# mulns/AccFlow

Measured on AMD Instinct MI355X. Metric: frame-pairs/s (estimator pair-evals/s), AccFlow(RAFT) 7-frame 480x1024 backward accumulation, higher is better.
Workload: dtype f32 (direct-kernel operands split into 2 fp16 terms - activations kept pre-split in HBM as fp16 hi+lo, 4 B per element; other kernels 3 bf16 terms; f32 accumulate); 1 GPU; AccFlow(RAFT) 7-frame 480x1024, 12 GRU iters, 1 sequence(s)/GPU/step (BASELINE.json configs[2]; configs[3] when n_gpus=8); parallelism=1 rank, no process group: no collective runs, weights=deterministic random init (no checkpoints offline)

## Files before the change

### accflow_amd/backward.py

```python
import torch

from . import _lib, ops, profiler
from .ops import _check, _p, _plane4, _stream


def _chw(t):
    return t.shape[1] * t.shape[2] * t.shape[3]


def act_backward(dy, y, act, out=None):
    lib = _lib.load()
    if out is None:
        out = torch.empty(tuple(dy.shape), dtype=torch.float32, device=dy.device)
    if tuple(dy.shape) != tuple(y.shape) or tuple(out.shape) != tuple(y.shape):
        raise RuntimeError("act_backward: shapes differ")
    _check(lib.accflow_act_backward_f32(_p(dy), _plane4(dy, "dy"), _p(y), _plane4(y, "y"), _p(out), _plane4(out, "dx"),
                                        dy.shape[0], _chw(dy), int(act), _stream()), "accflow_act_backward_f32")
    return out


def add_(dst, src):
    lib = _lib.load()
    if tuple(dst.shape) != tuple(src.shape):
        raise RuntimeError("add_: shapes differ")
    _check(lib.accflow_add_f32(_p(dst), _plane4(dst, "dst"), _p(src), _plane4(src, "src"), dst.shape[0], _chw(dst), _stream()),
           "accflow_add_f32")
    return dst


def l1_grad(pred, gt, scale):
    lib = _lib.load()
    pred, gt = ops._dense(pred, "pred"), ops._dense(gt, "gt")
    out = torch.empty_like(pred)
    _check(lib.accflow_l1_grad_f32(_p(pred), _p(gt), _p(out), pred.numel(), float(scale), _stream()), "accflow_l1_grad_f32")
    return out


def blend_backward(dy, f1, f2, m):
    lib = _lib.load()
    dy, f1, f2, m = (ops._dense(t, n) for t, n in ((dy, "dy"), (f1, "f1"), (f2, "f2"), (m, "m")))
    B, C, H, W = f1.shape
    df1, df2 = torch.empty_like(f1), torch.empty_like(f1)
    dm = torch.empty((B, 1, H, W), dtype=torch.float32, device=f1.device)
    _check(lib.accflow_blend_backward_f32(_p(dy), _p(f1), _p(f2), _p(m), _p(df1), _p(df2), _p(dm), B, C, H * W, _stream()),
           "accflow_blend_backward_f32")
    return df1, df2, dm


def convex_upsample_backward(dup, flow, mask):
    lib = _lib.load()
    dup, flow, mask = ops._dense(dup, "dup"), ops._dense(flow, "flow"), ops._dense(mask, "mask")
    B, _, H8, W8 = flow.shape
    if tuple(dup.shape) != (B, 2, 8 * H8, 8 * W8) or tuple(mask.shape) != (B, 576, H8, W8):
        raise RuntimeError("convex_upsample_backward: dup (B,2,8H8,8W8), mask (B,576,H8,W8)")
    dflow, dmask = torch.empty_like(flow), torch.empty_like(mask)
    _check(lib.accflow_convex_upsample_backward_f32(_p(dup), _p(flow), _p(mask), _p(dflow), _p(dmask), B, H8, W8, _stream()),
           "accflow_convex_upsample_backward_f32")
    return dflow, dmask


def conv_wgrad(x, dy, KH, KW, stride=1, padding=(0, 0), bias=True):
    lib = _lib.load()
    xbs, dbs = _plane4(x, "x"), _plane4(dy, "dy")
    B, Cin, H, W = x.shape
    Cout = dy.shape[1]
    pH, pW = (padding, padding) if isinstance(padding, int) else padding
    OH, OW = (H + 2 * pH - KH) // stride + 1, (W + 2 * pW - KW) // stride + 1
    if tuple(dy.shape) != (B, Cout, OH, OW):
        raise RuntimeError("conv_wgrad: dy is %s, expected %s" % (tuple(dy.shape), (B, Cout, OH, OW)))
    dw = torch.empty((Cout, Cin, KH, KW), dtype=torch.float32, device=x.device)
    db = torch.empty((Cout,), dtype=torch.float32, device=x.device) if bias else None
    tm = profiler.ACTIVE
    t0 = tm.begin() if tm is not None and tm.wants("conv_wgrad") else None
    _check(lib.accflow_conv_wgrad_f32(_p(x), xbs, _p(dy), dbs, _p(dw), _p(db), B, Cin, Cout, H, W, KH, KW, int(stride), int(pH),
                                      int(pW), _stream()), "accflow_conv_wgrad_f32")
    if t0 is not None:
        tm.end("conv_wgrad", t0, 2.0 * Cout * Cin * KH * KW * B * OH * OW, "wgrad Cin%d Cout%d k%dx%d s%d B%d %dx%d" % (
            Cin, Cout, KH, KW, stride, B, H, W))
    return dw, db


GRAD_CONV_MODE = "bf16x6"

_DGRAD_CACHE = {}


def _cached(deps, tag, build):
    if deps is None:
        return build()
    key = (tag, tuple(id(d) for d in deps))
    sig = tuple((d.data_ptr(), d._version, str(d.device)) for d in deps)
    hit = _DGRAD_CACHE.get(key)
    if hit is None or hit[0] != sig:
        hit = _DGRAD_CACHE[key] = [sig, build()]
    return hit[1]


def conv_dgrad(dy, weight, in_hw, stride=1, padding=(0, 0), out=None, deps=None):
    lib = _lib.load()
    pH, pW = (padding, padding) if isinstance(padding, int) else padding
    H, W = in_hw
    B = dy.shape[0]
    if callable(weight):
        weight = _cached(deps, "w", weight)
    Cout, Cin, KH, KW = weight.shape
    pad = (KH - 1 - pH, KW - 1 - pW)
    def make_pack():
        if ops.PACK_FUSED and Cin > 4:
            return ops.PackedConv(weight.detach().float(), None, stride=1, padding=pad, transpose_flip=True)
        return ops.PackedConv(weight.detach().float().transpose(0, 1).flip(2, 3).contiguous(), None, stride=1, padding=pad)
    pk = _cached(deps, ("pk", pad), make_pack)
    if stride != 1:
        Hd, Wd = H + 2 * pH - KH + 1, W + 2 * pW - KW + 1
        OH, OW = dy.shape[2:]
        g = torch.empty((B, Cout, Hd, Wd), dtype=torch.float32, device=dy.device)
        _check(lib.accflow_dilate_f32(_p(dy), _plane4(dy, "dy"), _p(g), B, Cout, OH, OW, Hd, Wd, int(stride), _stream()),
               "accflow_dilate_f32")
        dy = g
    with ops.conv_mode(GRAD_CONV_MODE):
        dx = ops.conv2d(pk, dy, out=out)
    if tuple(dx.shape[2:]) != (H, W):
        raise RuntimeError("conv_dgrad: got %s for an input of %s" % (tuple(dx.shape), (H, W)))
    return dx


def deform_conv_backward(x, offset, mask, weight, dy, need_dx=True, deps=None):
    lib = _lib.load()
    B, C, H, W = x.shape
    Cout, _, KH, KW = weight.shape
    T = KH * KW
    pH, pW = (KH - 1) // 2, (KW - 1) // 2
    cols = torch.empty((B, T * C, H, W), dtype=torch.float32, device=x.device)
    _check(lib.accflow_deform_columns_f32(_p(x), _plane4(x, "x"), _p(offset), _plane4(offset, "offset"), _p(mask),
                                          _plane4(mask, "dmask"), _p(cols), B, C, H, W, KH, KW, pH, pW, _stream()),
           "accflow_deform_columns_f32")
    dwz, db = conv_wgrad(cols, dy, 1, 1)
    dweight = dwz.reshape(Cout, KH, KW, C).permute(0, 3, 1, 2).contiguous()
    dcols = conv_dgrad(dy, lambda: weight.detach().float().permute(0, 2, 3, 1).reshape(Cout, T * C, 1, 1), (H, W),
                       deps=deps)
    dx = torch.empty((B, C, H, W), dtype=torch.float32, device=x.device)
    doff = torch.empty((B, 2 * T, H, W), dtype=torch.float32, device=x.device)
    dmsk = torch.empty((B, T, H, W), dtype=torch.float32, device=x.device)
    _check(lib.accflow_deform_conv_backward_f32(_p(x), _plane4(x, "x"), _p(offset), _plane4(offset, "offset"), _p(mask),
                                                _plane4(mask, "dmask"), _p(dcols), _p(dx), _plane4(dx, "dx"), _p(doff),
                                                _p(dmsk), B, C, H, W, KH, KW, pH, pW, _stream()),
           "accflow_deform_conv_backward_f32")
    return (dx if need_dx else None), doff, dmsk, dweight, db
```

### accflow_amd/csrc/conv2d_direct_kernel.h

```cpp
#pragma once
#include "conv_common.h"
#include <utility>

namespace {


#ifndef ACCFLOW_DIRECT_LEAN
#define ACCFLOW_DIRECT_LEAN 1
#endif
#ifndef ACCFLOW_DIRECT_LEAN_MAXSTEPS
#define ACCFLOW_DIRECT_LEAN_MAXSTEPS 0
#endif
#ifndef ACCFLOW_F16_PAIRMASK
#define ACCFLOW_F16_PAIRMASK 7
#endif
#ifndef ACCFLOW_DIRECT_KT_BUPFRONT
#define ACCFLOW_DIRECT_KT_BUPFRONT 0
#endif
#ifndef ACCFLOW_DIRECT_KT_WAVES
#define ACCFLOW_DIRECT_KT_WAVES 3
#endif
#ifndef ACCFLOW_DIRECT_SETPRIO
#define ACCFLOW_DIRECT_SETPRIO 0
#endif
template <class F, int... I>
__device__ __forceinline__ void dir_static_for_impl(std::integer_sequence<int, I...>, F&& f) {
  (f(std::integral_constant<int, I>{}), ...);
}
template <int N, class F>
__device__ __forceinline__ void dir_static_for(F&& f) { dir_static_for_impl(std::make_integer_sequence<int, N>{}, f); }

typedef int s16m_i32x4 __attribute__((ext_vector_type(4)));
__device__ __forceinline__ void s16m_load_a(u32x4& dst, unsigned voff, s16m_i32x4 desc, int soff) {
  asm volatile("buffer_load_dwordx4 %0, %1, %2, %3 offen" : "=v"(dst) : "v"(voff), "s"(desc), "s"(soff) : "memory");
}
template <int N>
__device__ __forceinline__ void s16m_wait_vm() {
  asm volatile("s_waitcnt vmcnt(%0)" : : "n"(N) : "memory");
  __builtin_amdgcn_sched_barrier(0);
}
__device__ __forceinline__ void s16m_wait_vm_but(int n) {
#define S16M_W(N) case N: s16m_wait_vm<N>(); break;
  switch (n) {
    S16M_W(1) S16M_W(2) S16M_W(3) S16M_W(4) S16M_W(5) S16M_W(6) S16M_W(7) S16M_W(8) S16M_W(9) S16M_W(10)
    S16M_W(11) S16M_W(12) S16M_W(13) S16M_W(14) S16M_W(15) S16M_W(16) S16M_W(17) S16M_W(18) S16M_W(19) S16M_W(20)
    S16M_W(21) S16M_W(22) S16M_W(23) S16M_W(24) S16M_W(25) S16M_W(26) S16M_W(27) S16M_W(28) S16M_W(29) S16M_W(30)
    default: s16m_wait_vm<0>();
  }
#undef S16M_W
}

template <bool F16>
__device__ __forceinline__ f32x16 dir_mfma(bf16x8 a, bf16x8 b, f32x16 c) {
  if constexpr (F16) return __builtin_amdgcn_mfma_f32_32x32x16_f16(__builtin_bit_cast(f16x8, a), __builtin_bit_cast(f16x8, b), c, 0, 0, 0);
  else return __builtin_amdgcn_mfma_f32_32x32x16_bf16(a, b, c, 0, 0, 0);
}

template <bool F16, class PixMap>
__device__ __forceinline__ void conv_epilogue_tapgemm(const accflow_conv_desc& d, f32x16 (&acc)[1][4], int cblk0, int wave,
                                                      int lane, int tid, int OHW, PixMap pixmap, float* red) {
  typedef float f32x4_ __attribute__((ext_vector_type(4)));
  typedef float f32x2_ __attribute__((ext_vector_type(2)));
  typedef _Float16 f16x2_ __attribute__((ext_vector_type(2)));
  const int l31 = lane & 31, kh = lane >> 5, lh4 = kh * 4;
  const int rowbase = cblk0 + wave * 32;
  const int R = d.tg_rows;
  const __amdgpu_buffer_rsrc_t r_b = __builtin_amdgcn_make_buffer_rsrc(const_cast<float*>(d.bias ? d.bias : d.wscale16), 0,
                                                                      d.bias ? d.Cout * 4 : 0, 0x00020000);
  const __amdgpu_buffer_rsrc_t r_s = __builtin_amdgcn_make_buffer_rsrc(const_cast<float*>(d.wscale16), 0, d.CoutPad * 4, 0x00020000);
  f32x4_ bv[4], sv[4];
#pragma unroll
  for (int m = 0; m < 4; ++m) {
    const int off = (rowbase + 8 * m + lh4) * 4;
    bv[m] = __builtin_bit_cast(f32x4_, __builtin_amdgcn_raw_buffer_load_b128(r_b, off, 0, 0));
    sv[m] = __builtin_bit_cast(f32x4_, __builtin_amdgcn_raw_buffer_load_b128(r_s, off, 0, 0));
  }
  const long long step_bytes2 = 2LL * d.tg_coutpad * 16, term_bytes2 = (long long)(d.Cout >> 4) * step_bytes2;
  const __amdgpu_buffer_rsrc_t r_w2 = __builtin_amdgcn_make_buffer_rsrc(const_cast<void*>(d.tg_w16), 0,
                                                                       (int)(unsigned)(2 * term_bytes2), 0x00020000);
  const unsigned av2 = (unsigned)((kh * d.tg_coutpad + l31) * 16);
  bf16x8 a2[2][2];
#pragma unroll
  for (int s = 0; s < 2; ++s)
#pragma unroll
    for (int t = 0; t < 2; ++t)
      a2[s][t] = __builtin_bit_cast(bf16x8, __builtin_amdgcn_raw_buffer_load_b128(
                                               r_w2, (int)av2, (int)(unsigned)(t * term_bytes2 + ((rowbase >> 4) + s) * step_bytes2), 0));
  constexpr float ASC16 = (float)(1 << ACCFLOW_F16_ASHIFT);
  bool bad16 = false;
#pragma unroll
  for (int tp = 0; tp < 4; ++tp) {
    f32x16 z2;
#pragma unroll
    for (int r = 0; r < 16; ++r) z2[r] = 0.0f;
#pragma unroll
    for (int s = 0; s < 2; ++s) {
      unsigned hi[4], lo[4];
#pragma unroll
      for (int e2 = 0; e2 < 4; ++e2) {
        const int m = 2 * s + (e2 >> 1), q = (2 * e2) & 3;
        float va = fmaf(acc[0][tp][4 * m + q], sv[m][q], bv[m][q]) + 0.0f;
        float vb = fmaf(acc[0][tp][4 * m + q + 1], sv[m][q + 1], bv[m][q + 1]) + 0.0f;
        va = fmaxf(va, 0.0f) * ASC16;
        vb = fmaxf(vb, 0.0f) * ASC16;
        bad16 |= !(va < 65520.0f) | !(vb < 65520.0f);
        const f32x2_ v2 = {va, vb};
        const f16x2_ hq = __builtin_convertvector(v2, f16x2_);
        const f32x2_ back = __builtin_convertvector(hq, f32x2_);
        const f32x2_ rest = {va - back[0], vb - back[1]};
        const f16x2_ lq = __builtin_convertvector(rest, f16x2_);
        hi[e2] = __builtin_bit_cast(unsigned, hq);
        lo[e2] = __builtin_bit_cast(unsigned, lq);
      }
      const u32x4 hv = {hi[0], hi[1], hi[2], hi[3]}, lv = {lo[0], lo[1], lo[2], lo[3]};
      const bf16x8 bh = __builtin_bit_cast(bf16x8, hv), bl = __builtin_bit_cast(bf16x8, lv);
      z2 = dir_mfma<F16>(a2[s][1], bh, z2);
      z2 = dir_mfma<F16>(a2[s][0], bl, z2);
      z2 = dir_mfma<F16>(a2[s][0], bh, z2);
    }
#pragma unroll
    for (int r = 0; r < 16; ++r) {
      const int row = 8 * (r >> 2) + lh4 + (r & 3);
      if (row < R) red[(wave * R + row) * (DIR_TH * DIR_TW) + tp * 32 + l31] = z2[r];
    }
  }
  if (bad16 && d.guard) atomicOr(d.guard, 1);
  __syncthreads();
  const long long obase = (long long)(cblk0 >> 7) * d.tg_out_ps;
  constexpr int NPX = DIR_TH * DIR_TW;
  for (int o = tid; o < R * NPX; o += 256) {
    const int row = o / NPX, px = o - row * NPX;
    const float v = ((red[o] + red[R * NPX + o]) + red[2 * R * NPX + o]) + red[3 * R * NPX + o];
    int b;
    const int rem = pixmap(px, b);
    if (rem >= 0) d.tg_out[obase + (long long)b * d.tg_out_bs + (long long)row * OHW + rem] = v * d.tg_scale[row];
  }
}

constexpr int DIR_NORM_MAXC = 256;
template <int TC, int NT, bool F16 = false, bool W4 = false, bool NORM = false, bool S16 = false, int PM = 7, bool TG = false, int KT = 0,
          int KWC = 0>
__global__ __launch_bounds__(256, (KT == 5 ? ACCFLOW_DIRECT_KT_WAVES : 2)) void conv2d_direct_bf16s_kernel(const accflow_conv_desc d) {
  static_assert(!F16 || NT == 2, "the fp16 split has two terms");
  static_assert(KT == 0 || ((S16 || (F16 && NORM)) && (KT & 1)), "the tap-specialised loop: S16 sources or the fp16 normalise-on-load gather, an odd tap count");
  static_assert(!TG || (W4 && S16 && PM == 7), "ACCFLOW_EPI_TAPGEMM: the 4 x 1 wave layout over S16 sources");
  static_assert(!W4 || TC == 2, "the 4 x 1 wave layout is the 128-channel kernel's");
  static_assert(!S16 || (F16 && !NORM), "S16 sources hold the fp16 split");
#ifdef ACCFLOW_KPROF
  const unsigned long long tL0 = __builtin_amdgcn_s_memrealtime();
  unsigned long long kp[8] = {0, 0, 0, 0, 0, 0, 0, 0};
#endif
  constexpr int WC = W4 ? 4 : 2, WP = W4 ? 1 : 2, TP = W4 ? 4 : 2, OCT = 2;
  constexpr int TCW = W4 ? 1 : TC;
  constexpr int BC = WC * TCW * 32;
  static_assert(BC == 2 * TC * 32 && DIR_TH * DIR_TW == WP * TP * 32, "4 x 32 pixel tile = 128 accumulator columns");
  constexpr int PSTAGE = NT * OCT * DIR_NPMAX;
  constexpr int TGWORDS = TG ? 4 * ACCFLOW_TAPGEMM_MAXROWS * DIR_TH * DIR_TW / 4 : 0;
  __shared__ u32x4 Pst[2 * PSTAGE > TGWORDS ? 2 * PSTAGE : TGWORDS];
  __shared__ float Nrm[NORM ? 2 * DIR_NORM_MAXC : 2];

  const int tid = threadIdx.x, lane = tid & 63;
  const int wave = __builtin_amdgcn_readfirstlane(tid >> 6);
  const int wc = wave / WP, wp = wave % WP;
  const int l31 = lane & 31, kh = lane >> 5;
  int bx = blockIdx.x, by = blockIdx.y;
#if ACCFLOW_CONV_XCD_ORDER
  if (gridDim.y > 1 && (d.C0 + d.C1) * d.KH * d.KW >= ACCFLOW_CONV_XCD_MIN_K) {
    const int X = gridDim.x, Y = gridDim.y, L = bx + X * by, full = X & ~7;
    if (L < full * Y) {
      const int G = L / (8 * Y), r = L - G * 8 * Y;
      by = r >> 3;
      bx = G * 8 + (r & 7);
    } else {
      const int r = L - full * Y, rem = X - full;
      by = r / rem;
      bx = full + r - by * rem;
    }
  }
#endif
  const int cblk0 = by * BC;
  const int OHW = d.OH * d.OW;
  const int tilesX = (d.OW + DIR_TW - 1) / DIR_TW, tilesY = (d.OH + DIR_TH - 1) / DIR_TH;
  const int tb = bx / (tilesX * tilesY), trem = bx - tb * tilesX * tilesY;
  const int oy0 = (trem / tilesX) * DIR_TH, ox0 = (trem % tilesX) * DIR_TW;
#ifdef ACCFLOW_DIRECT_STAGGER
  if (KT == 5 && (blockIdx.x & 1)) {
    for (int i = 0; i < ACCFLOW_DIRECT_STAGGER; ++i) __builtin_amdgcn_s_sleep(127);
  }
#endif
  const int T = d.KH * d.KW;
  const int PW = DIR_TW + d.KW - 1, NP = (DIR_TH + d.KH - 1) * PW;
  const int Cin = d.C0 + d.C1;
  const bool wide = T == 1;
  const int CCH = wide ? 32 : 16;
  const int NOCT = wide ? 4 : 2;
  const int NPS = wide ? DIR_NPMAX / 2 : DIR_NPMAX;
  const int TPC = wide ? 2 : T;
  const int nstep = (Cin + 15) / 16 * T, nchunk = (Cin + CCH - 1) / CCH;
  const int HW = d.H * d.W;
  const int c_begin = (int)((long long)nchunk * blockIdx.z / gridDim.z);
  const int c_end = (int)((long long)nchunk * (blockIdx.z + 1) / gridDim.z);
  const int step_end = min(c_end * TPC, nstep);

  unsigned voff0[2], voff1[2];
  int p_oct[2], p_pix[2];
#pragma unroll
  for (int i = 0; i < 2; ++i) {
    const int it = tid + 256 * i;
    const bool live = it < NOCT * NP;
    p_oct[i] = live ? it / NP : 0;
    p_pix[i] = live ? it - p_oct[i] * NP : 0;
    const int py = p_pix[i] / PW, px = p_pix[i] - py * PW;
    const int iy = oy0 - d.padH + py, ix = ox0 - d.padW + px;
    const bool ok = live && (unsigned)iy < (unsigned)d.H && (unsigned)ix < (unsigned)d.W;
    voff0[i] = ok ? (unsigned)(((long long)tb * d.in0_bs + iy * d.W + ix) * 4) : 0xFFFFFFFFu;
    voff1[i] = ok ? (unsigned)(((long long)tb * d.in1_bs + iy * d.W + ix) * 4) : 0xFFFFFFFFu;
    if (!live) p_pix[i] = -1;
  }
  const __amdgpu_buffer_rsrc_t rsrc0 = __builtin_amdgcn_make_buffer_rsrc(
      const_cast<float*>(d.in0), 0, (int)(unsigned)((((long long)(d.B - 1)) * d.in0_bs + (long long)d.C0 * HW) * 4),
      0x00020000);
  const __amdgpu_buffer_rsrc_t rsrc1 = __builtin_amdgcn_make_buffer_rsrc(
      const_cast<float*>(d.in1 ? d.in1 : d.in0), 0,
      (int)(unsigned)(d.in1 ? (((long long)(d.B - 1)) * d.in1_bs + (long long)d.C1 * HW) * 4 : 0), 0x00020000);
  unsigned pixo[4] = {0xFFFFFFFFu, 0xFFFFFFFFu, 0xFFFFFFFFu, 0xFFFFFFFFu};
  const int O0 = (d.C0 + 7) >> 3, O1 = (d.C1 + 7) >> 3;
  const __amdgpu_buffer_rsrc_t rs16_0 = __builtin_amdgcn_make_buffer_rsrc(
      const_cast<float*>(d.in0), 0, (int)(unsigned)((((long long)(d.B - 1)) * d.in0_bs + (long long)O0 * 2 * HW * 4) * 4),
      0x00020000);
  const __amdgpu_buffer_rsrc_t rs16_1 = __builtin_amdgcn_make_buffer_rsrc(
      const_cast<float*>(d.in1 ? d.in1 : d.in0), 0,
      (int)(unsigned)(d.in1 ? (((long long)(d.B - 1)) * d.in1_bs + (long long)O1 * 2 * HW * 4) * 4 : 0), 0x00020000);
  if constexpr (S16) {
#pragma unroll
    for (int q = 0; q < 4; ++q) {
      const int pp = q * 64 + lane;
      const int py = pp / PW, px = pp - py * PW;
      const int iy = oy0 - d.padH + py, ix = ox0 - d.padW + px;
      const bool ok = pp < NP && (unsigned)iy < (unsigned)d.H && (unsigned)ix < (unsigned)d.W;
      pixo[q] = ok ? (unsigned)(iy * d.W + ix) * 16u : 0xFFFFFFFFu;
    }
  }
  auto issue_dma = [&](int stage, int cc) {
    const int c0 = cc * CCH;
    const bool second = c0 >= d.C0;
    const int cs = second ? c0 - d.C0 : c0, osrc = second ? O1 : O0;
    const long long bs = second ? d.in1_bs : d.in0_bs;
    const unsigned item = (unsigned)((long long)tb * bs * 4);
#pragma unroll
    for (int i = 0; i < 4; ++i) {
      const int row = wide ? 2 * wave + (i >> 1) : wave;
      const int q = wide ? (i & 1) : i;
      if (!wide && q * 64 >= NP) continue;
      const int t = wide ? row >> 2 : row >> 1, o = wide ? row & 3 : row & 1;
      const int oct = (cs >> 3) + o;
      const unsigned soff = (unsigned)__builtin_amdgcn_readfirstlane((int)(item + (unsigned)((oct * 2 + t) * HW) * 16u));
      const unsigned voff = oct < osrc ? (q == 0 ? pixo[0] : q == 1 ? pixo[1] : q == 2 ? pixo[2] : pixo[3]) : 0xFFFFFFFFu;
      const int slot = __builtin_amdgcn_readfirstlane(stage * PSTAGE + t * (OCT * DIR_NPMAX) + o * NPS + q * 64);
      if (second)
        __builtin_amdgcn_raw_ptr_buffer_load_lds(rs16_1, (__attribute__((address_space(3))) void*)&Pst[slot], 16, (int)voff,
                                                 (int)soff, 0, 0);
      else
        __builtin_amdgcn_raw_ptr_buffer_load_lds(rs16_0, (__attribute__((address_space(3))) void*)&Pst[slot], 16, (int)voff,
                                                 (int)soff, 0, 0);
    }
  };
  float xa[8], xb[8];
  unsigned vq0[2], vq1[2];
#pragma unroll
  for (int i = 0; i < 2; ++i) {
    const unsigned po = (unsigned)p_oct[i] * 8u * (unsigned)HW * 4u;
    vq0[i] = voff0[i] != 0xFFFFFFFFu ? voff0[i] + po : 0xFFFFFFFFu;
    vq1[i] = voff1[i] != 0xFFFFFFFFu ? voff1[i] + po : 0xFFFFFFFFu;
  }
  auto gather_patch = [&](int cc) {
    const int c0 = cc * CCH;
    const bool second = c0 >= d.C0;
    const __amdgpu_buffer_rsrc_t rs = second ? rsrc1 : rsrc0;
    const int cs = second ? c0 - d.C0 : c0, cmax = second ? d.C1 : d.C0;
    if (cs + CCH <= cmax) {
      const unsigned va = second ? vq1[0] : vq0[0], vb = second ? vq1[1] : vq0[1];
      const unsigned so = (unsigned)__builtin_amdgcn_readfirstlane(cs) * (unsigned)HW * 4u;
#pragma unroll
      for (int q = 0; q < 8; ++q) {
        const int sq = (int)(so + (unsigned)q * (unsigned)HW * 4u);
        xa[q] = __builtin_bit_cast(float, __builtin_amdgcn_raw_buffer_load_b32(rs, (int)va, sq, 0));
        xb[q] = __builtin_bit_cast(float, __builtin_amdgcn_raw_buffer_load_b32(rs, (int)vb, sq, 0));
      }
      return;
    }
#pragma unroll
    for (int q = 0; q < 8; ++q) {
      const int ca = cs + p_oct[0] * 8 + q, cb = cs + p_oct[1] * 8 + q;
      const unsigned va = second ? voff1[0] : voff0[0], vb = second ? voff1[1] : voff0[1];
      const unsigned oa = (ca < cmax && va != 0xFFFFFFFFu) ? va + (unsigned)ca * (unsigned)HW * 4u : 0xFFFFFFFFu;
      const unsigned ob = (cb < cmax && vb != 0xFFFFFFFFu) ? vb + (unsigned)cb * (unsigned)HW * 4u : 0xFFFFFFFFu;
      xa[q] = __builtin_bit_cast(float, __builtin_amdgcn_raw_buffer_load_b32(rs, (int)oa, 0, 0));
      xb[q] = __builtin_bit_cast(float, __builtin_amdgcn_raw_buffer_load_b32(rs, (int)ob, 0, 0));
    }
  };
  bool bad = false;
  constexpr float ASC = (float)(1 << ACCFLOW_F16_ASHIFT);
  if constexpr (NORM) {
    for (int i = tid; i < 2 * d.C0; i += 256) Nrm[i] = d.in_norm[(long long)tb * 2 * d.C0 + i];
    __syncthreads();
  }
  auto store_patch = [&](int stage, int cc) {
    if constexpr (NORM) {
      const int ca = cc * CCH + p_oct[0] * 8, cb = cc * CCH + p_oct[1] * 8;
      const bool ina = voff0[0] != 0xFFFFFFFFu, inb = voff0[1] != 0xFFFFFFFFu;
#pragma unroll
      for (int q = 0; q < 8; ++q) {
        const bool oka = ina && ca + q < d.C0, okb = inb && cb + q < d.C0;
        const float ma = Nrm[2 * min(ca + q, d.C0 - 1)], ra = Nrm[2 * min(ca + q, d.C0 - 1) + 1];
        const float mb = Nrm[2 * min(cb + q, d.C0 - 1)], rb = Nrm[2 * min(cb + q, d.C0 - 1) + 1];
        xa[q] = oka ? fmaxf((xa[q] - ma) * ra, 0.0f) : 0.0f;
        xb[q] = okb ? fmaxf((xb[q] - mb) * rb, 0.0f) : 0.0f;
      }
    }
    u32x4 terms[NT];
    if constexpr (F16) split8_f16<0>(xa, terms, bad, ASC);
    else split8_bf16<NT, 0>(xa, terms);
    if (p_pix[0] >= 0) {
#pragma unroll
      for (int t = 0; t < NT; ++t) Pst[stage * PSTAGE + t * (OCT * DIR_NPMAX) + p_oct[0] * NPS + p_pix[0]] = terms[t];
    }
    if constexpr (F16) split8_f16<0>(xb, terms, bad, ASC);
    else split8_bf16<NT, 0>(xb, terms);
    if (p_pix[1] >= 0) {
#pragma unroll
      for (int t = 0; t < NT; ++t) Pst[stage * PSTAGE + t * (OCT * DIR_NPMAX) + p_oct[1] * NPS + p_pix[1]] = terms[t];
    }
  };

  const long long step_bytes = 2LL * d.CoutPad * 16, term_bytes = (long long)nstep * step_bytes;
  const __amdgpu_buffer_rsrc_t rsrcw = __builtin_amdgcn_make_buffer_rsrc(const_cast<void*>(F16 ? d.wpatch16 : d.wpatch), 0,
                                                                        (int)(unsigned)(3 * term_bytes), 0x00020000);
  const unsigned avoff = (unsigned)((kh * d.CoutPad + cblk0 + wc * TCW * 32 + l31) * 16);
#define DIR_LOAD_A(STEP, A)                                                                                      \
  _Pragma("unroll") for (int t = 0; t < NT; ++t) _Pragma("unroll") for (int tc = 0; tc < TCW; ++tc)              \
      A[t][tc] = __builtin_bit_cast(bf16x8, __builtin_amdgcn_raw_buffer_load_b128(                              \
          rsrcw, (int)(avoff + tc * 512), (int)(unsigned)(t * term_bytes + (STEP) * step_bytes), 0))

  int pbase[TP];
#pragma unroll
  for (int tp = 0; tp < TP; ++tp) pbase[tp] = (wp * TP + tp) * PW + l31;

  f32x16 acc[TCW][TP];
#pragma unroll
  for (int tc = 0; tc < TCW; ++tc)
#pragma unroll
    for (int tp = 0; tp < TP; ++tp)
#pragma unroll
      for (int r = 0; r < 16; ++r) acc[tc][tp][r] = 0.0f;

  bf16x8 aA[NT][TCW], aB[NT][TCW];
  DIR_LOAD_A(c_begin * TPC, aA);
  if constexpr (S16) {
    issue_dma(c_begin & 1, c_begin);
    asm volatile("s_waitcnt vmcnt(0)" ::: "memory");
  } else {
    gather_patch(c_begin);
    store_patch(c_begin & 1, c_begin);
  }
  __syncthreads();

  int cc = c_begin, tap = 0, ty = 0, tx = 0;
#define DIR_STEP(STEP, ACUR, ANXT)                                                                               \
  do {                                                                                                           \
    KPROF_T(tA);                                                                                                 \
    const int pstage = cc & 1;                                                                                   \
    const bool next_chunk = cc + 1 < c_end;                                                                      \
    if ((STEP) + 1 < step_end) { DIR_LOAD_A((STEP) + 1, ANXT); }                                                 \
    if (tap == 0 && next_chunk) {                                                                                \
      if constexpr (S16) issue_dma(pstage ^ 1, cc + 1); else gather_patch(cc + 1);                               \
    }                                                                                                            \
    KPROF_T(tA1);                                                                                                \
    const int toff = wide ? tap * 2 * NPS : ty * PW + tx;                                                        \
    bf16x8 b[NT][TP];                                                                                            \
    _Pragma("unroll") for (int t = 0; t < NT; ++t) _Pragma("unroll") for (int tp = 0; tp < TP; ++tp)             \
        b[t][tp] = __builtin_bit_cast(bf16x8, Pst[pstage * PSTAGE + t * (OCT * DIR_NPMAX) + kh * NPS + pbase[tp] + toff]); \
    KPROF_T(tB);                                                                                                 \
    KPROF_WAIT();                                                                                                \
    KPROF_T(tB2);                                                                                                \
    {                                                                                                            \
      if (ACCFLOW_DIRECT_SETPRIO) __builtin_amdgcn_s_setprio(ACCFLOW_DIRECT_SETPRIO);                            \
      constexpr int NPAIR = NT == 3 ? 6 : 3;                                                                     \
      constexpr int PA[6] = {2, 0, 1, 1, 0, 0}, PB[6] = {0, 2, 1, 0, 1, 0};                                      \
      _Pragma("unroll") for (int pr = 6 - NPAIR; pr < 6; ++pr) _Pragma("unroll") for (int tc = 0; tc < TCW; ++tc) \
          _Pragma("unroll") for (int tp = 0; tp < TP; ++tp) if (!F16 || (((ACCFLOW_F16_PAIRMASK & PM) >> (pr - 3)) & 1))  \
              acc[tc][tp] = dir_mfma<F16>(ACUR[PA[pr]][tc], b[PB[pr]][tp], acc[tc][tp]);                         \
      if (ACCFLOW_DIRECT_SETPRIO) __builtin_amdgcn_s_setprio(0);                                                 \
    }                                                                                                            \
    KPROF_T(tC);                                                                                                 \
    if (++tx == d.KW) { tx = 0; ++ty; }                                                                          \
    if (++tap == TPC || (STEP) + 1 == step_end) {                                                                \
      if constexpr (S16) { asm volatile("s_waitcnt vmcnt(0)" ::: "memory"); }                                    \
      else { if (next_chunk) store_patch(pstage ^ 1, cc + 1); }                                                  \
      KPROF_T(tD);                                                                                               \
      __syncthreads();                                                                                           \
      KPROF_T(tE);                                                                                               \
      KPROF_ACC(3, tD - tC); KPROF_ACC(4, tE - tD);                                                              \
      tap = 0; ty = 0; tx = 0; ++cc;                                                                             \
    }                                                                                                            \
    KPROF_ACC(0, tA1 - tA); KPROF_ACC(7, tB - tA1); KPROF_ACC(1, tB2 - tB); KPROF_ACC(2, tC - tB2); KPROF_ACC(5, 1); \
  } while (0)

#ifdef ACCFLOW_KPROF
  const unsigned long long tK0 = __builtin_readcyclecounter();
  const unsigned long long tR0 = __builtin_amdgcn_s_memrealtime();
  if (tid == 0) KP_SLOT(14) = tR0 - tL0;
#endif
  if constexpr (KT > 0) {
    static_assert(KWC > 0 && KT % KWC == 0, "the tap-specialised loop knows the kernel's width");
    constexpr int PWC_ = DIR_TW + KWC - 1;
    s16m_i32x4 wdesc;
    {
      const unsigned long long wp_ = (unsigned long long)(F16 ? d.wpatch16 : d.wpatch);
      wdesc[0] = (int)(unsigned)wp_;
      wdesc[1] = (int)(unsigned)((wp_ >> 32) & 0xFFFFu);
      wdesc[2] = (int)(unsigned)(3 * term_bytes);
      wdesc[3] = 0x00020000;
    }
    constexpr int NPC = (DIR_TH + KT / KWC - 1) * PWC_;
    constexpr int NDMA = !S16 ? 16 : (NPC + 63) / 64 < 4 ? (NPC + 63) / 64 : 4;
    auto load_a_asm = [&](int step, bf16x8 (&A)[NT][TCW]) __attribute__((always_inline)) {
#pragma unroll
      for (int t = 0; t < NT; ++t)
#pragma unroll
        for (int tc = 0; tc < TCW; ++tc)
        {
          u32x4 frag;
          s16m_load_a(frag, avoff + tc * 512, wdesc,
                      __builtin_amdgcn_readfirstlane((int)(unsigned)(t * term_bytes + (long long)step * step_bytes)));
          A[t][tc] = __builtin_bit_cast(bf16x8, frag);
        }
    };
    constexpr int PWC = DIR_TW + KWC - 1;
    const u32x4* const pb0 = &Pst[kh * DIR_NPMAX + wp * TP * PWC + l31];
    auto chunk = [&](int cq, bf16x8 (&A0)[NT][TCW], bf16x8 (&A1)[NT][TCW]) __attribute__((always_inline)) {
      const int pstage = cq & 1;
      const bool next_chunk = cq + 1 < c_end;
      const int sbase = cq * KT;
      const u32x4* const pb = pb0 + pstage * PSTAGE;
      dir_static_for<KT>([&](auto tap_) {
        constexpr int TAP = decltype(tap_)::value;
        bf16x8 (&ACUR)[NT][TCW] = (TAP & 1) ? A1 : A0;
        bf16x8 (&ANXT)[NT][TCW] = (TAP & 1) ? A0 : A1;
        const int snext = sbase + TAP + 1;
        if constexpr (TAP + 1 < KT) { load_a_asm(snext, ANXT); }
        else { if (next_chunk) { load_a_asm(snext, ANXT); } }
        if constexpr (TAP == 0) {
          if (next_chunk) {
            if constexpr (S16) issue_dma(pstage ^ 1, cq + 1);
            else gather_patch(cq + 1);
          }
        }
        bf16x8 b[NT][TP];
#pragma unroll
        for (int tt = 0; tt < NT; ++tt)
#pragma unroll
          for (int tp = 0; tp < TP; ++tp)
            b[tt][tp] = __builtin_bit_cast(bf16x8, pb[tt * (OCT * DIR_NPMAX) + tp * PWC + (TAP / KWC) * PWC + TAP % KWC]);
        constexpr int PA[3] = {1, 0, 0}, PB[3] = {0, 1, 0};
#pragma unroll
        for (int pr = 0; pr < 3; ++pr)
#pragma unroll
          for (int tc = 0; tc < TCW; ++tc)
#pragma unroll
            for (int tp = 0; tp < TP; ++tp) acc[tc][tp] = dir_mfma<F16>(ACUR[PA[pr]][tc], b[PB[pr]][tp], acc[tc][tp]);
#if ACCFLOW_DIRECT_KT_BUPFRONT
        __builtin_amdgcn_sched_group_barrier(0x100, NT * TP, 0);
        __builtin_amdgcn_sched_group_barrier(0x008, 3 * TCW * TP, 0);
#endif
        __builtin_amdgcn_sched_barrier(0);
        if constexpr (TAP == 0 && KT > 1) { if (next_chunk) s16m_wait_vm<NDMA>(); else s16m_wait_vm<0>(); }
        else if constexpr (TAP + 1 < KT) { s16m_wait_vm<0>(); }
      });
      s16m_wait_vm<0>();
      if constexpr (!S16) { if (next_chunk) store_patch(pstage ^ 1, cq + 1); }
      __syncthreads();
    };
    for (int cq = c_begin; cq < c_end; cq += 2) {
      chunk(cq, aA, aB);
      if (cq + 1 < c_end) chunk(cq + 1, aB, aA);
    }
  } else {
  for (int step = c_begin * TPC; step < step_end; step += 2) {
    DIR_STEP(step, aA, aB);
    if (step + 1 < step_end) DIR_STEP(step + 1, aB, aA);
  }
  }
#undef DIR_STEP
#undef DIR_LOAD_A
#ifdef ACCFLOW_KPROF
  {
    const unsigned long long tK1 = __builtin_readcyclecounter();
    if (tid == 0) {
      for (int i = 0; i < 6; ++i) KP_SLOT(i) = kp[i];
      KP_SLOT(6) = tK1 - tK0;
      KP_SLOT(7) = kp[7];
      KP_SLOT(8) = __builtin_amdgcn_s_memrealtime() - tR0;
      KP_SLOT(10) = 1;
    }
  }
#endif
  if constexpr (F16) {
    if (bad && d.guard) atomicOr(d.guard, 1);
  }
  auto pixmap = [&](int j, int& b) {
    const int oy = oy0 + j / DIR_TW, ox = ox0 + j % DIR_TW;
    b = tb;
    return (oy < d.OH && ox < d.OW) ? oy * d.OW + ox : -1;
  };
  if constexpr (TG) {
    conv_epilogue_tapgemm<F16>(d, acc, cblk0, wave, lane, tid, OHW, pixmap, reinterpret_cast<float*>(Pst));
    return;
  }
  if (gridDim.z > 1) {
    accflow_conv_desc e = d;
    e.out = d.kws + (long long)blockIdx.z * d.B * d.Cout * OHW;
    e.out_bs = (long long)d.Cout * OHW;
    e.bias = nullptr;
    e.wscale16 = nullptr;
    e.out16 = nullptr;
    e.cb = 0;
    conv_epilogue_impl<ACCFLOW_EPI_STORE, ACCFLOW_ACT_NONE, WC, WP, TCW, TP>(e, acc, cblk0, wc, wp, lane, OHW, pixmap);
    return;
  }
  if constexpr (S16) {
    if ((ACCFLOW_DIRECT_LEAN || d.p32 || nstep <= ACCFLOW_DIRECT_LEAN_MAXSTEPS) && d.epi == ACCFLOW_EPI_STORE && !d.cb && !d.stats && cblk0 + (wc + 1) * TCW * 32 <= d.Cout &&
        (d.act == ACCFLOW_ACT_NONE || d.act == ACCFLOW_ACT_RELU)) {
      if (d.act == ACCFLOW_ACT_RELU) conv_epilogue_lean<ACCFLOW_ACT_RELU, WC, WP, TCW, TP>(d, acc, cblk0, wc, wp, lane, OHW, pixmap);
      else conv_epilogue_lean<ACCFLOW_ACT_NONE, WC, WP, TCW, TP>(d, acc, cblk0, wc, wp, lane, OHW, pixmap);
      return;
    }
  }
#ifdef ACCFLOW_DIRECT_ABL_NOEPI
  if ((d.epi == ACCFLOW_EPI_GRU_ZR || d.epi == ACCFLOW_EPI_GRU_Q) && acc[0][0][0] != 12345.678f) return;
#endif
  if constexpr (S16 && W4 && KT == 5) {
    if (d.e0_fmt) {
      if (d.epi == ACCFLOW_EPI_GRU_ZR) conv_epilogue_gru16<true, TP>(d, acc, cblk0, wc, lane, OHW, pixmap);
      else conv_epilogue_gru16<false, TP>(d, acc, cblk0, wc, lane, OHW, pixmap);
      return;
    }
  }
  conv_epilogue_px<WC, WP, TCW, TP, decltype(pixmap), F16>(d, acc, cblk0, wc, wp, lane, OHW, pixmap, tb, trem * WP + wp);
#ifdef ACCFLOW_KPROF
  __builtin_amdgcn_sched_barrier(0);
  const unsigned long long tS = __builtin_amdgcn_s_memrealtime();
  asm volatile("s_waitcnt vmcnt(0)" ::: "memory");
  if (tid == 0) {
    KP_SLOT(15) = tS - tL0;
    KP_SLOT(11) = __builtin_amdgcn_s_memrealtime() - tL0;
  }
#endif
}


}

int accflow_direct_launch_s16(const accflow_conv_desc& d, int tc, dim3 grid, hipStream_t st);
int accflow_direct_launch_s16tg(const accflow_conv_desc& d, dim3 grid, hipStream_t st);
int accflow_direct_launch_s16k9(const accflow_conv_desc& d, int tc, bool tapgemm, dim3 grid, hipStream_t st);
int accflow_direct_launch_s16k(const accflow_conv_desc& d, int kt, dim3 grid, hipStream_t st);
int accflow_direct_launch_f16(const accflow_conv_desc& d, int tc, bool w4, dim3 grid, hipStream_t st);
int accflow_direct_launch_f16_norm(const accflow_conv_desc& d, int tc, dim3 grid, hipStream_t st);
int accflow_direct_launch_bf16(const accflow_conv_desc& d, int tc, int nt, bool w4, dim3 grid, hipStream_t st);
int accflow_direct_launch_bf16_norm(const accflow_conv_desc& d, int tc, int nt, dim3 grid, hipStream_t st);
```

Before: 513.5 frame-pairs/s.

## Triple-buffer A-operand loads in the 3x3 direct conv tap loop

For the KT==9 S16 non-W4 direct conv path, the A-operand register prefetch goes from double to triple buffering. A new chunk3 loop loads the A fragment two taps ahead and relaxes the vmcnt waits to leave NA loads in flight, so more global-load latency is hidden behind MFMAs. This costs an extra set of A registers, which may lower occupancy. The change also adds default-off ablation macros (no-A, no-B, no-MFMA, no-epilogue) and makes the dgrad weight cache check weakrefs so that reused object ids cannot return a stale entry.

Measured after the change: 516.4 frame-pairs/s, median of 6. About the same (+0.6%).

```diff
diff --git a/accflow_amd/backward.py b/accflow_amd/backward.py
--- a/accflow_amd/backward.py
+++ b/accflow_amd/backward.py
@@ -1,3 +1,5 @@
+import weakref
+
 import torch
 
 from . import _lib, ops, profiler
@@ -91,8 +93,8 @@
     key = (tag, tuple(id(d) for d in deps))
     sig = tuple((d.data_ptr(), d._version, str(d.device)) for d in deps)
     hit = _DGRAD_CACHE.get(key)
-    if hit is None or hit[0] != sig:
-        hit = _DGRAD_CACHE[key] = [sig, build()]
+    if hit is None or hit[0] != sig or any(r() is not d for r, d in zip(hit[2], deps)):
+        hit = _DGRAD_CACHE[key] = [sig, build(), tuple(weakref.ref(d) for d in deps)]
     return hit[1]
 
 
diff --git a/accflow_amd/csrc/conv2d_direct_kernel.h b/accflow_amd/csrc/conv2d_direct_kernel.h
--- a/accflow_amd/csrc/conv2d_direct_kernel.h
+++ b/accflow_amd/csrc/conv2d_direct_kernel.h
@@ -22,6 +22,18 @@
 #endif
 #ifndef ACCFLOW_DIRECT_SETPRIO
 #define ACCFLOW_DIRECT_SETPRIO 0
+#endif
+#ifndef ACCFLOW_DIRECT_ABL9_NOEPI
+#define ACCFLOW_DIRECT_ABL9_NOEPI 0
+#endif
+#ifndef ACCFLOW_DIRECT_ABL9_NOA
+#define ACCFLOW_DIRECT_ABL9_NOA 0
+#endif
+#ifndef ACCFLOW_DIRECT_ABL9_NOB
+#define ACCFLOW_DIRECT_ABL9_NOB 0
+#endif
+#ifndef ACCFLOW_DIRECT_ABL9_NOMFMA
+#define ACCFLOW_DIRECT_ABL9_NOMFMA 0
 #endif
 template <class F, int... I>
 __device__ __forceinline__ void dir_static_for_impl(std::integer_sequence<int, I...>, F&& f) {
@@ -152,6 +164,7 @@
 #endif
   constexpr int WC = W4 ? 4 : 2, WP = W4 ? 1 : 2, TP = W4 ? 4 : 2, OCT = 2;
   constexpr int TCW = W4 ? 1 : TC;
+  constexpr int ADEPTH = (KT == 9 && S16 && !W4) ? 3 : 2;
   constexpr int BC = WC * TCW * 32;
   static_assert(BC == 2 * TC * 32 && DIR_TH * DIR_TW == WP * TP * 32, "4 x 32 pixel tile = 128 accumulator columns");
   constexpr int PSTAGE = NT * OCT * DIR_NPMAX;
@@ -354,8 +367,9 @@
 #pragma unroll
       for (int r = 0; r < 16; ++r) acc[tc][tp][r] = 0.0f;
 
-  bf16x8 aA[NT][TCW], aB[NT][TCW];
+  bf16x8 aA[NT][TCW], aB[NT][TCW], aC[NT][TCW];
   DIR_LOAD_A(c_begin * TPC, aA);
+  if constexpr (ADEPTH == 3) { DIR_LOAD_A(c_begin * TPC + 1, aB); }
   if constexpr (S16) {
     issue_dma(c_begin & 1, c_begin);
     asm volatile("s_waitcnt vmcnt(0)" ::: "memory");
@@ -448,7 +462,9 @@
         bf16x8 (&ACUR)[NT][TCW] = (TAP & 1) ? A1 : A0;
         bf16x8 (&ANXT)[NT][TCW] = (TAP & 1) ? A0 : A1;
         const int snext = sbase + TAP + 1;
-        if constexpr (TAP + 1 < KT) { load_a_asm(snext, ANXT); }
+        constexpr bool ABL_A = KT == 9 && ACCFLOW_DIRECT_ABL9_NOA;
+        if constexpr (ABL_A) {}
+        else if constexpr (TAP + 1 < KT) { load_a_asm(snext, ANXT); }
         else { if (next_chunk) { load_a_asm(snext, ANXT); } }
         if constexpr (TAP == 0) {
           if (next_chunk) {
@@ -461,14 +477,21 @@
         for (int tt = 0; tt < NT; ++tt)
 #pragma unroll
           for (int tp = 0; tp < TP; ++tp)
-            b[tt][tp] = __builtin_bit_cast(bf16x8, pb[tt * (OCT * DIR_NPMAX) + tp * PWC + (TAP / KWC) * PWC + TAP % KWC]);
+            b[tt][tp] = (KT == 9 && ACCFLOW_DIRECT_ABL9_NOB)
+                            ? ACUR[tt][0]
+                            : __builtin_bit_cast(bf16x8, pb[tt * (OCT * DIR_NPMAX) + tp * PWC + (TAP / KWC) * PWC + TAP % KWC]);
         constexpr int PA[3] = {1, 0, 0}, PB[3] = {0, 1, 0};
 #pragma unroll
         for (int pr = 0; pr < 3; ++pr)
 #pragma unroll
           for (int tc = 0; tc < TCW; ++tc)
 #pragma unroll
-            for (int tp = 0; tp < TP; ++tp) acc[tc][tp] = dir_mfma<F16>(ACUR[PA[pr]][tc], b[PB[pr]][tp], acc[tc][tp]);
+            for (int tp = 0; tp < TP; ++tp) {
+              if constexpr (KT == 9 && ACCFLOW_DIRECT_ABL9_NOMFMA)
+                acc[tc][tp][pr] += __builtin_bit_cast(float, __builtin_bit_cast(u32x4, ACUR[PA[pr]][tc])[0] ^
+                                                                 __builtin_bit_cast(u32x4, b[PB[pr]][tp])[1]);
+              else acc[tc][tp] = dir_mfma<F16>(ACUR[PA[pr]][tc], b[PB[pr]][tp], acc[tc][tp]);
+            }
 #if ACCFLOW_DIRECT_KT_BUPFRONT
         __builtin_amdgcn_sched_group_barrier(0x100, NT * TP, 0);
         __builtin_amdgcn_sched_group_barrier(0x008, 3 * TCW * TP, 0);
@@ -481,9 +504,59 @@
       if constexpr (!S16) { if (next_chunk) store_patch(pstage ^ 1, cq + 1); }
       __syncthreads();
     };
-    for (int cq = c_begin; cq < c_end; cq += 2) {
-      chunk(cq, aA, aB);
-      if (cq + 1 < c_end) chunk(cq + 1, aB, aA);
+    auto chunk3 = [&](int cq) __attribute__((always_inline)) {
+      const int pstage = cq & 1;
+      const bool next_chunk = cq + 1 < c_end;
+      const int sbase = cq * KT;
+      const u32x4* const pb = pb0 + pstage * PSTAGE;
+      constexpr int NA = NT * TCW;
+      constexpr bool ABL_A = KT == 9 && ACCFLOW_DIRECT_ABL9_NOA;
+      dir_static_for<KT>([&](auto tap_) {
+        constexpr int TAP = decltype(tap_)::value;
+        bf16x8 (&ACUR)[NT][TCW] = TAP % 3 == 0 ? aA : TAP % 3 == 1 ? aB : aC;
+        bf16x8 (&AN2)[NT][TCW] = (TAP + 2) % 3 == 0 ? aA : (TAP + 2) % 3 == 1 ? aB : aC;
+        if constexpr (ABL_A) {}
+        else if constexpr (TAP + 2 < KT) { load_a_asm(sbase + TAP + 2, AN2); }
+        else { if (next_chunk) { load_a_asm(sbase + TAP + 2, AN2); } }
+        if constexpr (TAP == 0) {
+          if (next_chunk) issue_dma(pstage ^ 1, cq + 1);
+        }
+        bf16x8 b[NT][TP];
+#pragma unroll
+        for (int tt = 0; tt < NT; ++tt)
+#pragma unroll
+          for (int tp = 0; tp < TP; ++tp)
+            b[tt][tp] = (KT == 9 && ACCFLOW_DIRECT_ABL9_NOB)
+                            ? ACUR[tt][0]
+                            : __builtin_bit_cast(bf16x8, pb[tt * (OCT * DIR_NPMAX) + tp * PWC + (TAP / KWC) * PWC + TAP % KWC]);
+        constexpr int PA[3] = {1, 0, 0}, PB[3] = {0, 1, 0};
+#pragma unroll
+        for (int pr = 0; pr < 3; ++pr)
+#pragma unroll
+          for (int tc = 0; tc < TCW; ++tc)
+#pragma unroll
+            for (int tp = 0; tp < TP; ++tp) {
+              if constexpr (KT == 9 && ACCFLOW_DIRECT_ABL9_NOMFMA)
+                acc[tc][tp][pr] += __builtin_bit_cast(float, __builtin_bit_cast(u32x4, ACUR[PA[pr]][tc])[0] ^
+                                                                 __builtin_bit_cast(u32x4, b[PB[pr]][tp])[1]);
+              else acc[tc][tp] = dir_mfma<F16>(ACUR[PA[pr]][tc], b[PB[pr]][tp], acc[tc][tp]);
+            }
+        __builtin_amdgcn_sched_barrier(0);
+        if constexpr (ABL_A) { if constexpr (TAP + 1 < KT) s16m_wait_vm<0>(); }
+        else if constexpr (TAP == 0) { if (next_chunk) s16m_wait_vm<NA + NDMA>(); else s16m_wait_vm<NA>(); }
+        else if constexpr (TAP + 2 < KT) { s16m_wait_vm<NA>(); }
+        else if constexpr (TAP + 1 < KT) { if (next_chunk) s16m_wait_vm<NA>(); else s16m_wait_vm<0>(); }
+      });
+      if (next_chunk && !ABL_A) s16m_wait_vm<NA>(); else s16m_wait_vm<0>();
+      __syncthreads();
+    };
+    if constexpr (ADEPTH == 3) {
+      for (int cq = c_begin; cq < c_end; ++cq) chunk3(cq);
+    } else {
+      for (int cq = c_begin; cq < c_end; cq += 2) {
+        chunk(cq, aA, aB);
+        if (cq + 1 < c_end) chunk(cq + 1, aB, aA);
+      }
     }
   } else {
   for (int step = c_begin * TPC; step < step_end; step += 2) {
@@ -513,6 +586,9 @@
     b = tb;
     return (oy < d.OH && ox < d.OW) ? oy * d.OW + ox : -1;
   };
+  if constexpr (KT == 9 && ACCFLOW_DIRECT_ABL9_NOEPI) {
+    if (acc[0][0][0] != 12345.678f) return;
+  }
   if constexpr (TG) {
     conv_epilogue_tapgemm<F16>(d, acc, cblk0, wave, lane, tid, OHW, pixmap, reinterpret_cast<float*>(Pst));
     return;
```
